# tmkhang1999/TextMAE-Image-Compression

Measured on AMD Instinct MI355X. Metric: images/sec encode+decode+rate, ViT-B 256×256 batch64, 1/2/4/8 MI355X, higher is better.
Workload: dtype bf16; 1 GPU; MCM forward eval: ids+ViT-B/16 enc (K=144 of 256 patches) + LIC hyperprior + EB/GC rates + ViT dec 512/8/16 + unpatchify; img_size=256, num_keep_patches=144, per_gpu_batch=64, global_batch=64, parallelism=replicas x1, hip_graph=True

## Files before the change

include/tmae.h:

```cpp
#ifndef TMAE_H
#define TMAE_H

#include <stdint.h>

#ifdef __cplusplus
extern "C" {
#endif

#define TMAE_ABI_VERSION 1

enum { TMAE_OK = 0, TMAE_EINVAL = 1, TMAE_EHIP = 2 };
enum { TMAE_F32 = 0, TMAE_BF16 = 1 };
enum { TMAE_ACT_NONE = 0, TMAE_ACT_GELU = 1, TMAE_ACT_RELU = 2  };

const char* tmae_last_error_string(void);
int tmae_abi_version(void);

int tmae_ids_shuffle(const float* scores, int64_t* ids_shuffle, int64_t* ids_restore, int n, int L, int K,
                     int sum_lanes, void* stream);


int tmae_layernorm_fwd(const float* x, const float* gamma, const float* beta, void* y, int rows, int D,
                       int row_group, int group_stride, int row_offset, float eps, int out_dtype, void* stream);

// ... 41 lines not shown
  int cout, act, pixel_shuffle;
  void* y; int y_f32, ldy; long long y_s1, y_s2;
  float* y32; int ld32; long long y32_s1, y32_s2;
  const float* addend; int ld_add; long long a_s1, a_s2;
  const float* lrp_src; int ld_src; long long src_s1, src_s2;
  void* y2; int ldy2; long long y2_s1, y2_s2;
  int nb1, nb2;
  void* pre; int ldp; long long pre_s1, pre_s2;
} tmae_conv_args;
int tmae_conv3x3(const tmae_conv_args* args, int dtype, void* stream);

#define TMAE_LIC_STACK_MAXL 5
typedef struct tmae_lic_stack_args {
  int n, G, nb1, nb2, nlayers;
  const void* x1; int c1, ld1; long long x1_s[2];
  const void* x2; int c2, ld2; long long x2_s[2];
  const void* w[TMAE_LIC_STACK_MAXL]; long long w_s[TMAE_LIC_STACK_MAXL][2];
  const float* bias[TMAE_LIC_STACK_MAXL]; long long b_s[TMAE_LIC_STACK_MAXL][2];
  int cout[TMAE_LIC_STACK_MAXL];
  const float* addend; int ld_add; long long a_s[2];
  void* y; int y_f32, ldy; long long y_s[2];
  const float* lrp_src; int ld_src; long long src_s[2];
  void* y2; int ldy2; long long y2_s[2];
  int flags;
  int cn; const void* cw[TMAE_LIC_STACK_MAXL]; const float* cb[TMAE_LIC_STACK_MAXL]; int ccout[TMAE_LIC_STACK_MAXL];
  const void* cx1; int cc1, cld1;
  const float* yv; int ldyv;
  const float* cadd; int cld_add;
  float* csrc; int cld_src;
  void* cy; int cldy;
  void* cy2; int cldy2;
  long long cs_x1, cs_yv, cs_src, cs_add, cs_y, cs_y2, cs_w[TMAE_LIC_STACK_MAXL], cs_b[TMAE_LIC_STACK_MAXL];
  void* sv_pre[TMAE_LIC_STACK_MAXL]; void* sv_act[TMAE_LIC_STACK_MAXL]; long long sv_s[TMAE_LIC_STACK_MAXL][2];
  float* sv_t; long long sv_t_s[2];
  void* csv_pre[TMAE_LIC_STACK_MAXL]; void* csv_act[TMAE_LIC_STACK_MAXL]; long long cs_sv[TMAE_LIC_STACK_MAXL];
  float* csv_t; long long cs_t;
  float* racc[3]; int rld[3]; int rlim[3]; long long rs[3];
  const int* cq;
} tmae_lic_stack_args;
#define TMAE_LIC_STACK_CHAIN 1
#define TMAE_LIC_STACK_BWD 2
int tmae_lic_stack(const tmae_lic_stack_args* args, void* stream);

#define TMAE_LIC_LATENT_MAXP 4
typedef struct tmae_lic_latent_args {
  int n, G, cin, nb;
  const void* x[TMAE_LIC_LATENT_MAXP]; int ldx;
  const void* w; int nfr; long long blk;
  int f_off[TMAE_LIC_LATENT_MAXP]; int f_lo, f_hi;
  float* y; int ldy;
  long long y_s[TMAE_LIC_LATENT_MAXP];
  const float* bias[TMAE_LIC_LATENT_MAXP];
  int act, y_bf16;
} tmae_lic_latent_args;
int tmae_lic_latent(const tmae_lic_latent_args* args, void* stream);

int tmae_gc_slices_fwd(const float* y, int ldy, int yoff, const float* mu, const float* sigma, long long ms_stride,
                       int ld_ms, const float* noise, float* lik, int Mtot, void* yhat, int yhat_dtype, int ld_yhat,
                       float* yhat32, int ld32, int n, int HW, int nslices, int sw, void* stream);

int tmae_gc_slices_fwd_q(const float* y, int ldy, int yoff, const float* mu, const float* sigma, long long ms_stride,
                         int ld_ms, const float* noise, float* lik, int Mtot, void* yhat, int yhat_dtype, int ld_yhat,
                         float* yhat32, int ld32, int n, int HW, int nslices, int sw, float scale_bound, const int* q,
                         void* stream);

typedef struct tmae_eb_params {
  const float* matrix[5];
  const float* bias[5];
  const float* factor[4];
  const float* quantiles;
} tmae_eb_params;

int tmae_eb_likelihood_fwd(const float* z, const tmae_eb_params* params, const float* noise, float* lik,
                           void* zhat, int zhat_dtype, float* table, int n, int C, int HW, void* stream);

int tmae_eb_aux_loss(const tmae_eb_params* params, const float* target, float* out, float* table, int C,
                     void* stream);

int tmae_gc_likelihood_fwd(const float* x, const float* scales, const float* means, const float* noise,
                           float* x_tilde, float* lik, int total, float scale_bound, void* stream);

int tmae_bpp_sum(const float* y_lik, long long ny, const float* z_lik, long long nz, double* work, float* out,
                 double num_pixels, void* stream);

int tmae_nhwc_to_nchw(const float* x, int ldx, float* y, int n, int C, int HW, void* stream);

int tmae_crop_normalize_u8(const unsigned char* src, int nsrc, int H, int W, const int* crops, int B, int S,
                           const float* mean, const float* std, float* out, void* stream);

int tmae_mae_masking(const float* noise, int64_t* ids_shuffle, int64_t* ids_restore, float* mask, int n, int L,
                     int len_keep, void* stream);

int tmae_mae_loss(const float* pred, const float* imgs, const int64_t* ids_restore, int n, int C, int H, int W, int P,
                  int len_keep, int norm_pix_loss, double* work, float* out, void* stream);

int tmae_mae_loss_bwd(const float* pred, const float* imgs, const int64_t* ids_restore, int n, int C, int H, int W,
                      int P, int len_keep, int norm_pix_loss, const float* dloss, const float* dpred_in, void* out,
                      int out_dtype, void* stream);


int tmae_gc_slices_code(const float* y, int ldy, int yoff, const float* mu, const float* sigma, long long ms_stride,
                        int ld_ms, float* lik, int Mtot, void* yhat, int yhat_dtype, int ld_yhat, float* yhat32,
                        int ld32, int n, int HW, int nslices, int sw, int* symbols, int* indexes,
                        const float* scale_table, int nscale, void* stream);

int tmae_gc_indexes(const float* sigma, long long ms_stride, int ld_ms, int n, int HW, int nslices, int sw,
// ... 252 lines not shown
```

textmae-image-compression_amd/_lib.py:

```python
from __future__ import annotations

import ctypes
import os

PKG_DIR = os.path.dirname(os.path.abspath(__file__))
LIB_PATH = os.environ.get("TMAE_LIB") or os.path.join(PKG_DIR, "lib", "libtmae.so")

TMAE_F32, TMAE_BF16 = 0, 1
ACT_NONE, ACT_GELU, ACT_RELU = 0, 1, 2

P, I, F = ctypes.c_void_p, ctypes.c_int, ctypes.c_float


LL = ctypes.c_longlong


class ConvArgs(ctypes.Structure):
    _fields_ = [
        ("x1", P), ("c1", I), ("ld1", I), ("x1_s1", LL), ("x1_s2", LL),
        ("x2", P), ("c2", I), ("ld2", I), ("x2_s1", LL), ("x2_s2", LL),
        ("n", I), ("H", I), ("W", I), ("stride", I),
        ("w", P), ("w_s1", LL), ("w_s2", LL),
        ("bias", P), ("b_s1", LL), ("b_s2", LL),
        ("cout", I), ("act", I), ("pixel_shuffle", I),
# ... 24 lines not shown
class ConvDgradArgs(ctypes.Structure):
    _fields_ = [
        ("dy", P), ("ldy", I),
        ("n", I), ("H", I), ("W", I), ("stride", I), ("cout", I), ("cin", I),
        ("wd", P),
        ("out", P), ("out_f32", I), ("ldo", I), ("pre", P), ("ldp", I),
        ("acc", P * 3), ("ld_acc", I * 3), ("lim", I * 3),
        ("nb", I), ("s_dy", LL), ("s_wd", LL), ("s_out", LL), ("s_pre", LL),
    ]


LSTK_MAXL = 5


class LicStackArgs(ctypes.Structure):
    _fields_ = [
        ("n", I), ("G", I), ("nb1", I), ("nb2", I), ("nlayers", I),
        ("x1", P), ("c1", I), ("ld1", I), ("x1_s", LL * 2),
        ("x2", P), ("c2", I), ("ld2", I), ("x2_s", LL * 2),
        ("w", P * LSTK_MAXL), ("w_s", (LL * 2) * LSTK_MAXL),
        ("bias", P * LSTK_MAXL), ("b_s", (LL * 2) * LSTK_MAXL),
        ("cout", I * LSTK_MAXL),
        ("addend", P), ("ld_add", I), ("a_s", LL * 2),
        ("y", P), ("y_f32", I), ("ldy", I), ("y_s", LL * 2),
        ("lrp_src", P), ("ld_src", I), ("src_s", LL * 2),
        ("y2", P), ("ldy2", I), ("y2_s", LL * 2),
        ("flags", I),
        ("cn", I), ("cw", P * LSTK_MAXL), ("cb", P * LSTK_MAXL), ("ccout", I * LSTK_MAXL),
        ("cx1", P), ("cc1", I), ("cld1", I),
        ("yv", P), ("ldyv", I),
        ("cadd", P), ("cld_add", I),
        ("csrc", P), ("cld_src", I),
        ("cy", P), ("cldy", I),
        ("cy2", P), ("cldy2", I),
        ("cs_x1", LL), ("cs_yv", LL), ("cs_src", LL), ("cs_add", LL), ("cs_y", LL), ("cs_y2", LL),
        ("cs_w", LL * LSTK_MAXL), ("cs_b", LL * LSTK_MAXL),
        ("sv_pre", P * LSTK_MAXL), ("sv_act", P * LSTK_MAXL), ("sv_s", (LL * 2) * LSTK_MAXL),
        ("sv_t", P), ("sv_t_s", LL * 2),
        ("csv_pre", P * LSTK_MAXL), ("csv_act", P * LSTK_MAXL), ("cs_sv", LL * LSTK_MAXL),
        ("csv_t", P), ("cs_t", LL),
        ("racc", P * 3), ("rld", I * 3), ("rlim", I * 3), ("rs", LL * 3),
        ("cq", P),
    ]


class LicLatentArgs(ctypes.Structure):
    _fields_ = [
        ("n", I), ("G", I), ("cin", I), ("nb", I),
        ("x", P * 4), ("ldx", I),
        ("w", P), ("nfr", I), ("blk", LL),
        ("f_off", I * 4), ("f_lo", I), ("f_hi", I),
        ("y", P), ("ldy", I),
        ("y_s", LL * 4), ("bias", P * 4), ("act", I), ("y_bf16", I),
    ]


class EBParams(ctypes.Structure):
    _fields_ = [("matrix", ctypes.c_void_p * 5), ("bias", ctypes.c_void_p * 5), ("factor", ctypes.c_void_p * 4),
                ("quantiles", ctypes.c_void_p)]


SIGNATURES = {
    "tmae_abi_version": [],
    "tmae_ids_shuffle": [P, P, P, I, I, I, I, P],
    "tmae_layernorm_fwd": [P, P, P, P, I, I, I, I, I, F, I, P],
    "tmae_linear_fwd": [P, I, I, I, I, I, P, P, P, I, I, P, I, I, I, I, I, I, P],
    "tmae_linear_residual_fwd": [P, I, P, P, P, I, I, I, I, I, P],
    "tmae_patch_embed_fwd": [P, P, P, P, P, P, I, I, I, I, I, I, I, I, I, P],
    "tmae_patch_embed_gathered": [P, P, P, P, P, P, I, I, I, I, I, I, P],
    "tmae_cls_rows": [P, P, P, I, I, I, P],
    "tmae_mha_fwd": [P, P, I, I, I, I, F, I, P],
    "tmae_qkv_attn_fwd": [P, P, P, P, I, I, I, I, F, I, P],
    "tmae_decoder_embed_fwd": [P, I, P, P, P, P, P, I, I, I, I, I, I, P],
    "tmae_mask_rows": [P, P, P, P, I, I, I, I, P],
    "tmae_decoder_pred_fwd": [P, P, P, P, I, I, I, I, I, I, I, I, P],
    "tmae_decoder_pred_cp_fwd": [P, P, P, P, I, I, I, I, I, I, I, I, P],
    "tmae_conv3x3": [ctypes.POINTER(ConvArgs), I, P],
    "tmae_lic_stack": [ctypes.POINTER(LicStackArgs), P],
    "tmae_lic_latent": [ctypes.POINTER(LicLatentArgs), P],
    "tmae_gc_slices_fwd": [P, I, I, P, P, LL, I, P, P, I, P, I, I, P, I, I, I, I, I, P],
    "tmae_gc_slices_fwd_q": [P, I, I, P, P, LL, I, P, P, I, P, I, I, P, I, I, I, I, I, F, P, P],
    "tmae_eb_likelihood_fwd": [P, ctypes.POINTER(EBParams), P, P, P, I, P, I, I, I, P],
    "tmae_eb_aux_loss": [ctypes.POINTER(EBParams), P, P, P, I, P],
    "tmae_gc_likelihood_fwd": [P, P, P, P, P, P, I, F, P],
    "tmae_nhwc_to_nchw": [P, I, P, I, I, I, P],
    "tmae_crop_normalize_u8": [P, I, I, I, P, I, I, ctypes.POINTER(F), ctypes.POINTER(F), P, P],
    "tmae_bpp_sum": [P, LL, P, LL, P, P, ctypes.c_double, P],
    "tmae_gemm_plan": [I, I, I, I, I, ctypes.c_char_p, I],
    "tmae_mha_plan": [I, I, I, I, ctypes.c_char_p, I],
    "tmae_mae_masking": [P, P, P, P, I, I, I, P],
    "tmae_mae_loss": [P, P, P, I, I, I, I, I, I, I, P, P, P],
    "tmae_mae_loss_bwd": [P, P, P, I, I, I, I, I, I, I, P, P, P, I, P],
    "tmae_gc_slices_code": [P, I, I, P, P, LL, I, P, I, P, I, I, P, I, I, I, I, I, P, P, P, I, P],
    "tmae_gc_indexes": [P, LL, I, I, I, I, I, P, I, F, P, P],
    "tmae_gc_dequantize": [P, P, LL, I, I, I, I, I, I, P, I, I, P, I, P],
    "tmae_gc_slices_code_q": [P, I, I, P, P, LL, I, P, I, P, I, I, P, I, I, I, I, I, P, P, P, I, F, P, P],
    "tmae_gc_indexes_q": [P, LL, I, I, I, I, I, P, I, F, P, P, P],
    "tmae_gc_dequantize_q": [P, P, LL, I, I, I, I, I, I, P, I, I, P, I, P, P],
    "tmae_gc_slices_code_qm": [P, I, I, P, P, LL, I, P, I, P, I, I, P, I, I, I, I, I, P, P, P, I, F, P, P],
    "tmae_gc_indexes_qm": [P, LL, I, I, I, I, I, P, I, F, P, P, P],
    "tmae_gc_dequantize_qm": [P, P, LL, I, I, I, I, I, I, P, I, I, P, I, P, P],
    "tmae_gc_slices_fwd_qm": [P, I, I, P, P, LL, I, P, P, I, P, I, I, P, I, I, I, I, I, F, P, P],
    "tmae_gc_pmf": [P, P, I, I, P, P, P],
    "tmae_eb_pmf": [ctypes.POINTER(EBParams), P, P, I, I, P, P, P],
    "tmae_eb_symbols": [P, ctypes.POINTER(EBParams), P, I, I, I, P, P],
    "tmae_eb_dequantize": [P, ctypes.POINTER(EBParams), P, I, I, I, P, I, P],
# ... 122 lines not shown
```

textmae-image-compression_amd/csrc/lic_stack.hip:

```cpp
#include "lic_stack_kernel.h"

int lic_stack_launch_q(const tmae_lic_stack_args& a, int nwg, hipStream_t stream);

extern "C" int tmae_lic_stack(const tmae_lic_stack_args* args, void* stream) {
  using namespace lstk;
  TMAE_REQUIRE(args != nullptr, "tmae_lic_stack: args is NULL");
  const tmae_lic_stack_args& a = *args;
  TMAE_REQUIRE(a.G >= 1 && a.G * a.G <= MAXPIX, "tmae_lic_stack: grid %dx%d exceeds %d pixels", a.G, a.G, MAXPIX);
  TMAE_REQUIRE(a.nlayers >= 1 && a.nlayers <= TMAE_LIC_STACK_MAXL, "tmae_lic_stack: %d layers", a.nlayers);
  TMAE_REQUIRE(a.nb1 >= 1 && a.nb2 >= 1 && a.n >= 1, "tmae_lic_stack: batch %d x %d, n %d", a.nb1, a.nb2, a.n);
  const bool bwd = (a.flags & TMAE_LIC_STACK_BWD) != 0;
  TMAE_REQUIRE(!a.cq || (!bwd && (a.flags & TMAE_LIC_STACK_CHAIN)),
               "tmae_lic_stack: cq (the chain's quantiser step) needs TMAE_LIC_STACK_CHAIN and no TMAE_LIC_STACK_BWD");
  TMAE_REQUIRE(a.x1 != nullptr && (a.y != nullptr || bwd), "tmae_lic_stack: x1 / y required");
  if (bwd) {
    TMAE_REQUIRE(!(a.flags & TMAE_LIC_STACK_CHAIN) && !a.addend && !a.lrp_src && !a.x2 && !a.sv_t,
                 "tmae_lic_stack: the backward chain takes no chain / addend / lrp / second source");
    const bool rt = a.racc[0] != nullptr;
    for (int l = 0; l < a.nlayers; ++l)
      TMAE_REQUIRE(a.w[l] && ((rt && l + 1 == a.nlayers) || (a.sv_pre[l] && a.sv_act[l])),
                   "tmae_lic_stack: backward layer %d needs w / sv_pre / sv_act", l);
    if (rt) {
      const int cl = a.cout[a.nlayers - 1];
      TMAE_REQUIRE(a.nb2 <= 1, "tmae_lic_stack: routed accumulators need nb2 == 1 (got %d)", a.nb2);
      TMAE_REQUIRE(a.rlim[0] >= 0 && a.rlim[0] <= a.rlim[1] && a.rlim[1] <= a.rlim[2] && a.rlim[2] == cl &&
                   a.rlim[0] % 4 == 0 && a.rlim[1] % 4 == 0, "tmae_lic_stack: routes %d / %d / %d of %d channels",
                   a.rlim[0], a.rlim[1], a.rlim[2], cl);
      for (int r = 0; r < 3; ++r)
        TMAE_REQUIRE((r == 0 ? a.rlim[0] : a.rlim[r] - a.rlim[r - 1]) == 0 || (a.racc[r] && a.rld[r] % 4 == 0),
                     "tmae_lic_stack: route %d accumulator", r);
    }
  }
  TMAE_REQUIRE(a.c1 >= 0 && a.c2 >= 0 && (a.c2 == 0 || a.x2 != nullptr), "tmae_lic_stack: channels %d + %d", a.c1, a.c2);
  TMAE_REQUIRE(a.c1 % 8 == 0 && a.c2 % 8 == 0 && a.ld1 % 8 == 0 && (a.c2 == 0 || a.ld2 % 8 == 0),
               "tmae_lic_stack: input channels / strides must be multiples of 8");
  TMAE_REQUIRE(pad32(a.c1 + a.c2) <= MAXC, "tmae_lic_stack: %d input channels exceed %d", a.c1 + a.c2, MAXC);
  for (int l = 0; l < a.nlayers; ++l) {
    TMAE_REQUIRE((a.w[l] != nullptr || (l == 0 && a.c1 + a.c2 == 0)) && (a.bias[l] != nullptr || bwd),
                 "tmae_lic_stack: layer %d weights", l);
    TMAE_REQUIRE(a.cout[l] >= 4 && a.cout[l] % 8 == 0, "tmae_lic_stack: layer %d cout %d (multiple of 8)", l, a.cout[l]);
    TMAE_REQUIRE((l + 1 == a.nlayers && (!bwd || a.racc[0])) || pad32(a.cout[l]) <= MAXC,
                 "tmae_lic_stack: layer %d cout %d exceeds %d", l, a.cout[l], MAXC);
  }
  TMAE_REQUIRE(!a.lrp_src || !a.y_f32, "tmae_lic_stack: lrp output is bf16");
  if (a.flags & TMAE_LIC_STACK_CHAIN) {
    TMAE_REQUIRE(a.nb1 == 2 && a.y_f32 && !a.lrp_src && a.cn >= 1 && a.cn <= TMAE_LIC_STACK_MAXL,
                 "tmae_lic_stack: chain needs the 2 x nb2 mean / scale problems with f32 outputs");
    TMAE_REQUIRE(a.ccout[a.cn - 1] == a.cout[a.nlayers - 1] && a.cx1 && a.yv && a.csrc && a.cy,
                 "tmae_lic_stack: chain operands");
    TMAE_REQUIRE(a.cc1 % 8 == 0 && a.cld1 % 8 == 0 && a.ldyv % 4 == 0 && a.cld_src % 4 == 0 && a.ldy % 4 == 0 &&
                 pad32(a.cc1 + a.ccout[a.cn - 1]) <= MAXC, "tmae_lic_stack: chain channels %d + %d", a.cc1,
                 a.ccout[a.cn - 1]);
    for (int l = 0; l < a.cn; ++l)
      TMAE_REQUIRE(a.cw[l] && a.cb[l] && a.ccout[l] % 8 == 0 && (l + 1 == a.cn || pad32(a.ccout[l]) <= MAXC),
                   "tmae_lic_stack: chain layer %d", l);
  }
  if (a.addend) TMAE_REQUIRE(a.ld_add % 4 == 0, "tmae_lic_stack: addend stride %d", a.ld_add);
  for (int l = 0; l < a.nlayers; ++l)
    TMAE_REQUIRE(!a.sv_pre[l] == !a.sv_act[l], "tmae_lic_stack: layer %d keeps pre-activation and output together", l);
  for (int l = 0; l < a.cn && (a.flags & TMAE_LIC_STACK_CHAIN); ++l)
    TMAE_REQUIRE(!a.csv_pre[l] == !a.csv_act[l], "tmae_lic_stack: chain layer %d keeps pre and output together", l);
  TMAE_REQUIRE(!a.sv_t || a.lrp_src, "tmae_lic_stack: sv_t is the lrp stack's pre-tanh value");
  const int nwg = a.n * a.nb1 * a.nb2;
  if (bwd) hipLaunchKernelGGL((lic_stack_kernel<true, false>), dim3(nwg), dim3(NW * 64), 0, (hipStream_t)stream, a);
  else if (a.cq) return lic_stack_launch_q(a, nwg, (hipStream_t)stream);
  else hipLaunchKernelGGL((lic_stack_kernel<false, false>), dim3(nwg), dim3(NW * 64), 0, (hipStream_t)stream, a);
  TMAE_LAUNCH_CHECK("tmae_lic_stack");
}

namespace llat {
constexpr int NW = 8, FPW = 2 * NW;
constexpr int MAXCIN = 384;
constexpr unsigned PMAX = lstk::pitch(MAXCIN);
constexpr unsigned ZOFF = lstk::MAXPIX * PMAX;
constexpr unsigned TMASK = ZOFF + 16 * PMAX;
constexpr int LDS_BYTES = TMASK + 320;
}
__device__ __forceinline__ constexpr unsigned llat_zoff() { return llat::ZOFF; }
__device__ __forceinline__ constexpr unsigned llat_tmask() { return llat::TMASK; }

struct LlatOut {
  void* y;
  int ldy, bf, act;
  const float* bias;
};

template <int NKC>
__device__ __forceinline__ void llat_item(const bf16* w, int nfr, long long blk, int f0, int fcol, bool two,
                                          const unsigned char* lb, unsigned pin, int G, int npix, int img,
                                          const LlatOut& o, int lane) {
  constexpr int MF = 9, NS = 9 * NKC;
  constexpr int D = NKC % 4 == 0 ? 4 : NKC % 3 == 0 ? 3 : NKC % 2 == 0 ? 2 : (NKC <= 7 ? NKC : 1);
  asm volatile("" : "+v"(lane));
  const int fr = lane & 15, fq = lane >> 4;
  f32x4 acc[2][MF];
#pragma unroll
  for (int i = 0; i < 2; ++i)
#pragma unroll
    for (int j = 0; j < MF; ++j) acc[i][j] = f32x4{0.f, 0.f, 0.f, 0.f};
  const unsigned sstride = (unsigned)nfr * 512u;
  const bf16* wl[2];
  bf16x8 ar[D][2];
#pragma unroll
  for (int i = 0; i < 2; ++i) {
    const int f = two || i == 0 ? f0 + i : f0;
    const int b = f / nfr, fi = f - b * nfr;
    wl[i] = w + b * blk + ((size_t)fi * 64 + lane) * 8;
#pragma unroll
    for (int d = 0; d < D; ++d) {
      ar[d][i] = *reinterpret_cast<const bf16x8*>(wl[i]);
      wl[i] += sstride;
    }
  }
  unsigned tmask[MF];
#pragma unroll
  for (int j = 0; j < MF; ++j) tmask[j] = *reinterpret_cast<const unsigned short*>(lb + llat_tmask() + 2 * (16 * j + fr));
  auto row = [&](int t, int j) -> unsigned {
    const int p = 16 * j + fr, sh = (t / 3 - 1) * G + (t % 3 - 1);
    const unsigned r = (unsigned)(p + sh);
    return ((tmask[j] >> t) & 1u ? r * pin : llat_zoff() + (r & 15u) * pin) + 16u * fq;
  };
  bf16x8 bv[2][MF];
  unsigned rb[MF];
#pragma unroll
// ... 11 lines not shown
#pragma unroll
        for (int j = 0; j < MF; ++j) bv[(kc + 1) & 1][j] = *reinterpret_cast<const bf16x8*>(lb + rb[j] + 64u * (kc + 1));
      } else if (t + 1 < 9) {
#pragma unroll
        for (int j = 0; j < MF; ++j) bv[(kc + 1) & 1][j] = *reinterpret_cast<const bf16x8*>(lb + rn[j]);
      }
      bf16x8 a0[2];
      const bool more = t * NKC + kc + D < NS;
#pragma unroll
      for (int i = 0; i < 2; ++i) {
        a0[i] = ar[kc % D][i];
        if (more) {
          ar[kc % D][i] = *reinterpret_cast<const bf16x8*>(wl[i]);
          wl[i] += sstride;
        }
      }
#pragma unroll
      for (int j = 0; j < MF; ++j)
#pragma unroll
        for (int i = 0; i < 2; ++i)
          acc[i][j] = __builtin_amdgcn_mfma_f32_16x16x32_bf16(a0[i], bv[kc & 1][j], acc[i][j], 0, 0, 0);
      __builtin_amdgcn_sched_barrier(0);
    }
    if constexpr (NKC & 1) {
#pragma unroll
      for (int j = 0; j < MF; ++j) bv[0][j] = bv[1][j];
    }
#pragma unroll
    for (int j = 0; j < MF; ++j) rb[j] = rn[j];
  }
  f32x4 bias[2];
#pragma unroll
  for (int i = 0; i < 2; ++i)
    bias[i] = o.bias ? load4f(o.bias + fcol + 16 * (two ? i : 0) + 4 * fq) : f32x4{0.f, 0.f, 0.f, 0.f};
#pragma unroll
  for (int j = 0; j < MF; ++j) {
    const int p = 16 * j + fr;
    if (p >= npix) continue;
    const size_t at = ((size_t)img * npix + p) * o.ldy + fcol + 4 * fq;
#pragma unroll
    for (int i = 0; i < 2; ++i) {
      if (i == 1 && !two) break;
      f32x4 v = acc[i][j] + bias[i];
      if (o.act == TMAE_ACT_GELU) {
        const f32x2 lo = gelu2_bf16out(v.xy), hi = gelu2_bf16out(v.zw);
        v = f32x4{lo.x, lo.y, hi.x, hi.y};
      }
      if (o.bf) store4(reinterpret_cast<bf16*>(o.y) + at + 16 * i, v);
      else store4(reinterpret_cast<float*>(o.y) + at + 16 * i, v);
    }
  }
}

template <int NKC>
__global__ void __launch_bounds__(llat::NW * 64) lic_latent_kernel(tmae_lic_latent_args a) {
  using namespace llat;
  __shared__ __attribute__((aligned(16))) uint4 lds[LDS_BYTES / 16];
  unsigned char* lb = reinterpret_cast<unsigned char*>(lds);
  const int n = a.n, G = a.G, npix = G * G, cin = 32 * NKC;
  const int t = xcd_remap(blockIdx.x, gridDim.x);
  const int tile = t / n, img = t - tile * n, prob = blockIdx.y;
  const int tid = threadIdx.x, lane = tid & 63, wave = tid >> 6;
  const unsigned pin = lstk::pitch(cin);
  for (int i = tid; i < 16 * (int)pin / 16; i += NW * 64) reinterpret_cast<uint4*>(lds)[ZOFF / 16 + i] = uint4{0, 0, 0, 0};
  for (int p = tid; p < 160; p += NW * 64) {
    unsigned m = 0;
    if (p < npix) {
      const int py = p / G, px = p - py * G;
#pragma unroll
      for (int k = 0; k < 9; ++k) {
        const int yy = py + k / 3 - 1, xx = px + k % 3 - 1;
        m |= ((unsigned)yy < (unsigned)G && (unsigned)xx < (unsigned)G) ? (1u << k) : 0u;
      }
    }
    *reinterpret_cast<unsigned short*>(lb + TMASK + 2 * p) = (unsigned short)m;
  }
  {
    const bf16* x = reinterpret_cast<const bf16*>(a.x[prob]);
    constexpr int q = 4 * NKC;
    for (int i = tid; i < npix * q; i += NW * 64) {
      const int p = i / q, ch = 8 * (i - p * q);
      *reinterpret_cast<uint4*>(lb + p * pin + 2 * ch) =
          *reinterpret_cast<const uint4*>(x + ((size_t)img * npix + p) * a.ldx + ch);
    }
  }
  __syncthreads();
  const int fr0 = a.f_lo + tile * FPW + 2 * wave;
  if (fr0 >= a.f_hi) return;
  LlatOut o;
  o.ldy = a.ldy;
  o.bf = a.y_bf16;
  o.act = a.act;
  o.bias = a.bias[prob];
  o.y = a.y_bf16 ? (void*)(reinterpret_cast<bf16*>(a.y) + a.y_s[prob]) : (void*)(a.y + a.y_s[prob]);
  llat_item<NKC>(reinterpret_cast<const bf16*>(a.w), a.nfr, a.blk, a.f_off[prob] + fr0, 16 * fr0, fr0 + 1 < a.f_hi, lb,
                 pin, G, npix, img, o, lane);
}

extern "C" int tmae_lic_latent(const tmae_lic_latent_args* args, void* stream) {
  TMAE_REQUIRE(args != nullptr, "tmae_lic_latent: args is NULL");
  const tmae_lic_latent_args& a = *args;
  TMAE_REQUIRE(a.G >= 1 && a.G * a.G <= lstk::MAXPIX, "tmae_lic_latent: grid %dx%d", a.G, a.G);
  TMAE_REQUIRE(a.cin >= 32 && a.cin % 32 == 0 && a.cin <= llat::MAXCIN, "tmae_lic_latent: cin %d (multiple of 32, <= %d)",
               a.cin, llat::MAXCIN);
  TMAE_REQUIRE(a.nb >= 1 && a.nb <= TMAE_LIC_LATENT_MAXP && a.n >= 1, "tmae_lic_latent: %d problems, %d images", a.nb,
               a.n);
  TMAE_REQUIRE(a.w && a.y && a.ldx % 8 == 0 && a.ldx >= a.cin, "tmae_lic_latent: operands / strides");
  TMAE_REQUIRE(a.nfr >= 1 && a.f_lo >= 0 && a.f_hi > a.f_lo && a.f_lo % 2 == 0, "tmae_lic_latent: fragments [%d, %d) "
               "of blocks of %d (f_lo even)", a.f_lo, a.f_hi, a.nfr);
  TMAE_REQUIRE(a.blk >= 9LL * (a.cin / 32) * a.nfr * 512 || a.f_off[0] + a.f_hi <= a.nfr, "tmae_lic_latent: block stride");
  TMAE_REQUIRE(a.act == TMAE_ACT_NONE || a.act == TMAE_ACT_GELU, "tmae_lic_latent: act %d", a.act);
  TMAE_REQUIRE(a.ldy % 4 == 0 && (a.ldy >= 16 * a.f_hi), "tmae_lic_latent: ldy %d", a.ldy);
  for (int j = 0; j < a.nb; ++j)
    TMAE_REQUIRE(a.x[j] && a.f_off[j] >= 0 && a.y_s[j] % 4 == 0, "tmae_lic_latent: problem %d", j);
  const int ntile = (a.f_hi - a.f_lo + llat::FPW - 1) / llat::FPW;
  const dim3 grid(a.n * ntile, a.nb);
  hipStream_t st = (hipStream_t)stream;
  switch (a.cin / 32) {
#define LLAT_CASE(K) \
  case K: hipLaunchKernelGGL(lic_latent_kernel<K>, grid, dim3(llat::NW * 64), 0, st, a); break;
    LLAT_CASE(1) LLAT_CASE(2) LLAT_CASE(3) LLAT_CASE(4) LLAT_CASE(5) LLAT_CASE(6)
    LLAT_CASE(7) LLAT_CASE(8) LLAT_CASE(9) LLAT_CASE(10) LLAT_CASE(11) LLAT_CASE(12)
#undef LLAT_CASE
    default: break;
  }
  TMAE_LAUNCH_CHECK("tmae_lic_latent");
}
```

textmae-image-compression_amd/mcm.py:

```python
from __future__ import annotations

import collections.abc
import os

from functools import partial

import numpy as np
import torch
import torch.nn as nn

from . import ops
from .entropy import CompressionModel, EntropyBottleneck, GaussianConditional
from .layers import Block, BlockScratch, BlockWeights, PatchEmbed, conv3x3, run_block, subpel_conv3x3
from .pos_embed import get_2d_sincos_pos_embed


class MCM(CompressionModel):

    def __init__(self, img_size=224, patch_size=16, in_chans=3, encoder_embed_dim=768, encoder_depth=12,
                 encoder_num_heads=12, decoder_embed_dim=512, decoder_depth=8, decoder_num_heads=16, mlp_ratio=4.0,
                 norm_layer=partial(nn.LayerNorm, eps=1e-6), norm_pix_loss=False, latent_depth=384,
                 hyperprior_depth=192, num_slices=12, num_keep_patches=144):
        super().__init__()
        self.frozen_stages = -1
# ... 644 lines not shown
                s1 += 1
            part = [sections[j] for j in jobs[s0:s1]]
            try:
                x_hat = self._decode_sections([a[0] for a in part], [a[1] for a in part], [a[2] for a in part],
                                              lanes[0], lanes[1], who, [index[k].q for k, _ in jobs[s0:s1]],
                                              [(index[k].nlev, index[k].offsets, a[3])
                                               for (k, _), a in zip(jobs[s0:s1], part)])
            except ValueError as e:

                def name(m, s0=s0):
                    k, t = jobs[s0 + int(m.group(1))]
                    return f"tile {t} of source {where[k]}" if many else f"tile {t}"

                raise ValueError(re.sub(r"\bimage (\d+)", name, str(e), count=1)) from None
            if tiles is None:
                tiles = torch.empty((len(jobs),) + tuple(x_hat.shape[1:]), dtype=torch.float32, device=x_hat.device)
            tiles[s0:s1].copy_(x_hat)
            s0 = s1
        images = [(g.H, g.W, slots[k]) for k, g in enumerate(grids)]
        return ops.tile_blend_crops(tiles, images, windows, size, index[0].overlap, out=out)


class _LazyStreams(collections.abc.Mapping):

    def __init__(self, **tensors):
        self._t, self._h = tensors, {}

    def __getitem__(self, key):
        if key not in self._h:
            self._h[key] = self._t[key].cpu().numpy()
        return self._h[key]

    def __iter__(self):
        return iter(self._t)

    def __len__(self):
        return len(self._t)


def _interleave(layers):
    out = []
    for j, l in enumerate(layers):
        out.append(l)
        if j < len(layers) - 1:
            out.append(nn.GELU())
    return out


class _Executor:

    USE_LIC_STACK = True
    USE_LIC_CHAIN = True
    USE_LIC_LATENT = True

    def __init__(self, m: MCM, batch, dtype, device):
        self.m, self.batch, self.dtype, self.device = m, batch, dtype, device
        self._sig = None
        B = batch
        E, Dd, M, N, S = m.encoder_embed_dim, m.decoder_embed_dim, m.latent_depth, m.hyperprior_depth, m.num_slices
        K = m.num_keep_patches
        P = m.encoder_embed.patch_size[0]
        self.img = m.encoder_embed.img_size[0]
        self.P, self.L = P, m.encoder_embed.num_patches
        self.g = g = int(round(K ** 0.5))
        if g * g != K:
            raise ValueError(f"num_keep_patches={K} must be a perfect square (MCM.py:729-732 views it as sqrt x sqrt)")
        self.hz = ((g + 1) // 2 + 1) // 2
        if self.hz * 4 != g:
            raise ValueError(f"sqrt(num_keep_patches)={g} must be a multiple of 4 so h_s returns to the y grid")
        self.sw = M // S
        self.maxsup = S // 2
        gc = m.gaussian_conditional
        self.scale_bound = float(gc.scale_bound) if gc.scale_bound is not None else 0.11
        self.nb = S - self.maxsup
        f32, dt = torch.float32, dtype
        dev = device

        def z(*shape, dtype=f32):
            return torch.empty(shape, dtype=dtype, device=dev)

        Te, Td = K + 1, self.L + 1
        Mp = B * g * g
        self.Mp = Mp
        hid_e = m.encoder_blocks[0].mlp.fc1.out_features if m.encoder_depth else 4 * E
        hid_d = m.decoder_blocks[0].mlp.fc1.out_features if m.decoder_depth else 4 * Dd
        self.tok = z(B * Te, E)
        self.enc_s = BlockScratch(B * Te, E, hid_e, dt, dev)
        self.enc_out = z(B * K, E, dtype=dt)
        ga = [l.out_channels for l in m.g_a if isinstance(l, nn.Conv2d)]
        self.ga_buf = [z(B * K, c, dtype=dt) for c in ga[:-1]]
        self.Y32 = z(Mp, M)
        self.YT = self.Y32 if dt == f32 else z(Mp, M, dtype=dt)
        ha = [l.out_channels for l in m.h_a if isinstance(l, nn.Conv2d)]
        res = [g, g, (g + 1) // 2, (g + 1) // 2, self.hz]
        self.ha_buf = [z(B * r * r, c, dtype=dt) for c, r in zip(ha[:-1], res[:-1])]
        self.Z = z(B * self.hz * self.hz, N)
        self.ZLIK = z(B, N, self.hz, self.hz)
        self.ZHAT = z(B * self.hz * self.hz, N, dtype=dt)
        self.eb_table = z(N, 59)
        self.zero_loss = torch.zeros((), device=device)
        hs_out = [m.h_s_mean[0].out_channels, m.h_s_mean[2][0].out_channels // 4, m.h_s_mean[4].out_channels,
                  m.h_s_mean[6][0].out_channels // 4]
        hs_res = [self.hz, 2 * self.hz, 2 * self.hz, g]
        self.hs_buf = [z(2, B * r * r, c, dtype=dt) for c, r in zip(hs_out, hs_res)]
        self.LSM = z(2, Mp, M, dtype=dt)
        self.LS, self.LM = self.LSM[0], self.LSM[1]
        self.mid = [l.out_channels for l in m.cc_transform_mean[0] if isinstance(l, nn.Conv2d)]
        c0 = self.mid[0]
        self.PW = 3 * S * c0
        self.Pbuf = z(Mp, self.PW)
        self.overlap = torch.device(dev).type == "cuda"
        self.side_stream = torch.cuda.Stream(device=dev) if self.overlap else None
        self.SUPY = z(Mp, M, dtype=dt)
        self.YPRE = z(Mp, M)
        self.YH = z(Mp, M, dtype=dt)
        nb = self.nb
        self.CM = [z(2, nb, Mp, c, dtype=dt) for c in self.mid[:-1]]
        self.MUSIG = z(2, nb, Mp, self.sw)
        self.MS_SER = z(2, S, Mp, self.sw)
        self.CL = [z(nb, Mp, c, dtype=dt) for c in self.mid[:-1]]
        self.YLIK = z(B, M, g, g)
        gs = [l.out_channels for l in m.g_s if isinstance(l, nn.ConvTranspose2d)]
        self.gs_buf = [z(B * K, c, dtype=dt) for c in gs]
        self.dec = z(B * Td, Dd)
        self.dec_s = BlockScratch(B * Td, Dd, hid_d, dt, dev)
        self.dn = z(B * self.L, Dd, dtype=dt)

    def refresh_weights(self):
        sig = tuple((p.data_ptr(), p._version) for p in self.m.parameters())
        if sig == self._sig:
            return
        self._sig = sig
        m, dt = self.m, self.dtype
        M, S, sw, ms = m.latent_depth, m.num_slices, self.sw, self.maxsup

        def cast(t):
            t = t.detach()
            return (t if dt == torch.float32 else t.to(dt)).contiguous()

        def cw(w, lo=None, hi=None):
            w = w.detach()
            if lo is not None:
                w = w[:, lo:hi]
            return w.permute(0, 2, 3, 1).reshape(w.shape[0], -1)

        self.w_pe = cast(m.encoder_embed.proj.weight.view(m.encoder_embed.proj.weight.shape[0], -1))
        self.enc_w = [BlockWeights.from_block(b, dt) for b in m.encoder_blocks]
        self.dec_w = [BlockWeights.from_block(b, dt) for b in m.decoder_blocks]
        self.ga_w = [(cast(l.weight.view(l.weight.shape[0], -1)), l.bias.detach())
                     for l in m.g_a if isinstance(l, nn.Conv2d)]
        self.gs_w = [(cast(l.weight.view(l.weight.shape[0], -1).t()), l.bias.detach())
                     for l in m.g_s if isinstance(l, nn.ConvTranspose2d)]
        self.ha_w = [(cast(cw(l.weight)), l.bias.detach(), l.stride[0]) for l in m.h_a if isinstance(l, nn.Conv2d)]

        def hs_convs(seq):
            out = []
            for l in seq:
                if isinstance(l, nn.Conv2d):
                    out.append((l, False))
                elif isinstance(l, nn.Sequential):
                    out.append((l[0], True))
            return out

        self.hs2_w = [(cast(torch.stack([cw(s.weight), cw(mn.weight)])),
                       torch.stack([s.bias, mn.bias]).detach().contiguous(), ps)
# ... 478 lines not shown
                ops.gc_slices_code_q(self.Y32, M, i0 * sw, mu, sigma, ms_stride, sw, None, M, self.SUPY, dt, M,
                                     self.YPRE, M, B, HW, nbs, sw, sym[i0 * per:], idx[i0 * per:], table, bound, qd)
        return step

    def _gc_decompress(self, decoder):
        gc = self.m.gaussian_conditional
        M, sw, B, HW, dt = self.m.latent_depth, self.sw, self.batch, self.g * self.g, self.dtype
        cdf, sizes, offsets = gc.host_tables()
        bound = float(gc.scale_bound) if gc.scale_bound is not None else 0.11
        per = B * sw * HW
        idx_dev = torch.empty(self.m.num_slices * per, dtype=torch.int32, device=self.device)

        def step(i0, nbs, mu, sigma, ms_stride):
            n = nbs * per
            ops.gc_indexes(sigma, ms_stride, sw, B, HW, nbs, sw, gc.scale_table, bound, idx_dev)
            idx = idx_dev[:n].cpu().numpy()
            vals = decoder.decode_stream_array(idx, cdf, sizes, offsets)
            sym = torch.from_numpy(vals).to(self.device)
            ops.gc_dequantize(sym, mu, ms_stride, sw, B, HW, nbs, sw, i0 * sw, self.SUPY, dt, M, self.YPRE, M)
        return step

    def _h_s(self):
        B, dt = self.batch, self.dtype
        x, xs, cin, H = self.ZHAT, 0, self.m.hyperprior_depth, self.hz
        for j, (w, b, pshuf) in enumerate(self.hs2_w):
            last = j == len(self.hs2_w) - 1
            cout = w.shape[1]
            out = self.LSM if last else self.hs_buf[j]
            ops.conv3x3(x, cin, cin, B, H, H, w, b, out, out.shape[2], cout, dt,
                        act=ops.ACT_NONE if last else ops.ACT_GELU, pixel_shuffle=pshuf, nb=(1, 2),
                        strides={"x1": (0, xs), "w": (0, w[0].numel()), "b": (0, cout), "y": (0, out[0].numel())})
            if pshuf:
                H *= 2
                cin = cout // 4
            else:
                cin = cout
            x, xs = out, out[0].numel()

    def _slices(self, gc_step, chain_ok=False, cq=None):
        m, dt, B, g = self.m, self.dtype, self.batch, self.g
        M, S, sw, ms, nb, Mp = m.latent_depth, m.num_slices, self.sw, self.maxsup, self.nb, self.Mp
        mid = self.mid
        c0 = mid[0]
        Pw = self.PW
        Pb = self.Pbuf
        eP = Pb.element_size()
        pbase = Pb.data_ptr()
        off_mean, off_lrp, off_scale = 0, S * c0, 2 * S * c0
        esz = self.SUPY.element_size()
        supy, ypre, yh = self.SUPY.data_ptr(), self.YPRE.data_ptr(), self.YH.data_ptr()
        e4 = 4
        wrow = self.w_pre_ml[0].numel()

        def pre(i0, i1):
            if self.w_lat is not None:
                nfs = c0 // 16
                ops.lic_latent(B, g, [self.LM, self.LM, self.LS], M, M, self.w_lat, nfs, self.w_lat[0].numel(),
                               [0, S * nfs, 2 * S * nfs], i0 * nfs, i1 * nfs, pbase, Pw)
                return
            n = (i1 - i0) * c0
            ops.conv3x3(self.LM, M, M, B, g, g, self.w_pre_ml[i0 * c0:], None, pbase + (off_mean + i0 * c0) * eP, Pw,
                        n, dt, y_f32=True, nb=(1, 2), strides={"w": (0, S * c0 * wrow), "y": (0, S * c0)})
            ops.conv3x3(self.LS, M, M, B, g, g, self.w_pre_s[i0 * c0:], None, pbase + (off_scale + i0 * c0) * eP,
                        Pw, n, dt, y_f32=True)

        ready = {}
        groups = [(i, i + 1) for i in range(1, ms)] + ([(ms, S)] if nb > 0 else [])
        if self.overlap and groups:
            main = torch.cuda.current_stream()
            pre(0, 1)
            fork = torch.cuda.Event()
            fork.record(main)
            side = self.side_stream
            side.wait_event(fork)
            with torch.cuda.stream(side):
                for i0, i1 in groups:
                    pre(i0, i1)
                    ev = torch.cuda.Event()
                    ev.record(side)
                    ready[i0] = ev
        else:
            pre(0, S)

        def wait_pre(i0):
            if i0 in ready:
                torch.cuda.current_stream().wait_event(ready.pop(i0))

        cm = [t.data_ptr() for t in self.CM]
        cl = [t.data_ptr() for t in self.CL]
        musig = self.MUSIG.data_ptr()
        cm_s1 = [nb * Mp * c for c in mid[:-1]]
        ms_s1 = nb * Mp * sw

        def ms_stack(first, layers, x1, c1, i0, nbs):
            w, b = first
            ops.conv3x3(x1, c1, M, B, g, g, w, b, cm[0], c0, c0, dt, act=ops.ACT_GELU,
                        addend=pbase + (off_mean + i0 * c0) * eP, ld_add=Pw, nb=(2, nbs),
                        strides={"w": (w[0].numel(), w[0][0].numel() if nbs > 1 else 0),
                                 "b": (b[0].numel(), c0 if nbs > 1 else 0),
                                 "a": (off_scale - off_mean, c0), "y": (cm_s1[0], Mp * c0)})
            for j, (w, b) in enumerate(layers):
                cin, cout = mid[j], mid[j + 1]
                last = j == len(layers) - 1
                y = musig if last else cm[j + 1]
                ys1 = ms_s1 if last else cm_s1[j + 1]
                ops.conv3x3(cm[j], cin, cin, B, g, g, w, b, y, cout, cout, dt,
                            act=ops.ACT_NONE if last else ops.ACT_GELU, y_f32=last, nb=(2, nbs),
                            strides={"x1": (cm_s1[j], Mp * cin), "w": (w[0].numel(), w[0][0].numel() if nbs > 1 else 0),
                                     "b": (b[0].numel(), cout if nbs > 1 else 0), "y": (ys1, Mp * cout)})

        def ms_fused(i0, nbs):
            ws = self.lstk["b_ms"] if nbs > 1 else self.lstk["ms"][i0]
            first, layers = (self.b_ms_first, self.b_ms_layers) if nbs > 1 else (self.ms_first[i0], self.ms_layers[i0])
            bs_ = [first[1]] + [b for _, b in layers]
            st = {"a": (off_scale - off_mean, c0), "y": (ms_s1, Mp * sw)}
            for l, (w, b) in enumerate(zip(ws, bs_)):
                st[f"w{l}"] = (w[0].numel(), w[0][0].numel() if nbs > 1 else 0)
                st[f"b{l}"] = (b[0].numel(), b.shape[-1] if nbs > 1 else 0)
            ops.lic_stack(B, g, supy, sw * (ms if nbs > 1 else i0), M, ws, bs_, mid, musig, sw, True,
                          addend=pbase + (off_mean + i0 * c0) * eP, ld_add=Pw, nb=(2, nbs), strides=st)

        def lrp_fused(i0, nbs):
            ws = self.lstk["b_lrp"] if nbs > 1 else self.lstk["lrp"][i0]
            first, layers = (self.b_lrp_first, self.b_lrp_layers) if nbs > 1 else (self.lrp_first[i0], self.lrp_layers[i0])
            bs_ = [first[1]] + [b for _, b in layers]
            st = {"a": (0, c0), "y": (0, sw), "src": (0, sw), "x2": (0, sw)}
            for l, (w, b) in enumerate(zip(ws, bs_)):
                st[f"w{l}"] = (0, w[0].numel() if nbs > 1 else 0)
                st[f"b{l}"] = (0, b.shape[-1] if nbs > 1 else 0)
            if nbs > 1:
# ... 83 lines not shown
```

textmae-image-compression_amd/ops.py:

```python
from __future__ import annotations

import contextlib
import ctypes
import os

import torch

from . import _lib
from ._lib import ACT_GELU, ACT_NONE, TMAE_BF16, TMAE_F32, ConvArgs, EBParams, LicStackArgs

__all__ = [
    "ids_shuffle", "layernorm", "linear", "linear_residual", "patch_embed", "cls_rows", "mha", "decoder_embed",
    "mask_rows", "decoder_pred", "conv3x3", "lic_stack", "pack_lic_stack_weight", "lic_stack_fits", "gc_slices", "eb_likelihood", "eb_aux_loss",
    "gc_likelihood", "nhwc_to_nchw", "bpp", "gemm_plan", "force_gemm_tile", "GEMM_TILES", "mha_plan", "mha_force_stream", "dtype_code", "gc_slices_code", "gc_indexes",
    "gc_dequantize", "gc_slices_fwd_q", "gc_slices_code_q", "gc_indexes_q", "gc_dequantize_q",
    "gc_slices_fwd_qm", "gc_slices_code_qm", "gc_indexes_qm", "gc_dequantize_qm",
    "qlevels_select", "qlevels_pack", "qlevels_unpack", "qmap_build",
    "gc_pmf", "eb_pmf", "eb_symbols", "eb_dequantize", "invert_permutation", "mae_masking",
    "rans_stream_cap_words", "rans_encode_streams", "rans_pack_streams", "rans_decode_streams",
    "rans_encode_lanes", "rans_decode_lanes", "ids_pack", "ids_unpack",
    "resize_tables", "resize_u8", "rgb_to_gray_u8", "tile_cut_u8", "tile_blend", "tile_blend_crops",
    "mae_loss", "TMAE_F32", "TMAE_BF16", "ACT_NONE", "ACT_GELU",
]

# ... 237 lines not shown
    if ci:
        t[:, :co, :ci] = w.float().permute(2, 3, 0, 1).reshape(9, co, ci)
    nkc, nfr = cip // 32, cop // 16
    t = t.view(9, nfr, 16, nkc, 4, 8).permute(0, 3, 1, 4, 2, 5).contiguous()
    return t.view(-1).to(dtype)


def pack_lic_stack_weight_t(w: torch.Tensor, dtype=torch.bfloat16) -> torch.Tensor:
    return pack_lic_stack_weight(w.detach().transpose(0, 1).flip(2, 3), dtype)


def lic_stack_bwd(n, G, dtop, ldt, c_top, weights, couts, pres, outs, nb=(1, 1), strides=None, routes=None):
    a = LicStackArgs()
    if routes is not None:
        if nb[1] != 1:
            raise ValueError("lic_stack_bwd routes: nb2 must be 1")
        if len(routes) > 1 and len(routes) != nb[0]:
            raise ValueError("lic_stack_bwd routes: one route list per problem")
        lim = 0
        for r in range(3):
            if r < len(routes[0]):
                acc, ld, nc = routes[0][r]
                a.racc[r], a.rld[r] = _p(acc), ld
                if len(routes) > 1 and nc:
                    steps = [_p(routes[k + 1][r][0]) - _p(routes[k][r][0]) for k in range(len(routes) - 1)]
                    if len(set(steps)) != 1 or steps[0] % 4:
                        raise ValueError("lic_stack_bwd routes: accumulators not at a constant stride")
                    a.rs[r] = steps[0] // 4
                lim += nc
            a.rlim[r] = lim
    a.n, a.G, a.nlayers = n, G, len(couts)
    a.nb1, a.nb2 = nb
    a.x1, a.c1, a.ld1 = _p(dtop), c_top, ldt
    a.flags = 2
    for l, (w, c) in enumerate(zip(weights, couts)):
        a.w[l], a.cout[l] = _p(w), c
        if l < len(pres):
            a.sv_pre[l], a.sv_act[l] = _p(pres[l]), _p(outs[l])
    for name, (s1, s2) in (strides or {}).items():
        if name[0] == "w":
            a.w_s[int(name[1:])][:] = (s1, s2)
        elif name[0] == "s":
            a.sv_s[int(name[1:])][:] = (s1, s2)
        else:
            getattr(a, f"{name}_s")[:] = (s1, s2)
    _lib.call("tmae_lic_stack", ctypes.byref(a), _stream())


def lic_latent_fits(G, cin):
    return G * G <= LSTK_MAXPIX and cin % 32 == 0 and 32 <= cin <= 384


def lic_latent(n, G, xs, ldx, cin, w, nfr, blk, f_off, f_lo, f_hi, y, ldy, y_s=None, biases=None, act=ACT_NONE,
               y_bf16=False):
    a = _lib.LicLatentArgs()
    a.n, a.G, a.cin, a.nb = n, G, cin, len(xs)
    for j, (x, fo) in enumerate(zip(xs, f_off)):
        a.x[j] = _p(x)
        a.f_off[j] = fo
        a.y_s[j] = (16 * fo) if y_s is None else y_s[j]
        a.bias[j] = _p(biases[j]) if biases is not None else None
    a.ldx, a.w, a.nfr, a.blk = ldx, _p(w), nfr, blk
    a.f_lo, a.f_hi = f_lo, f_hi
    a.y, a.ldy = _p(y), ldy
    a.act, a.y_bf16 = act, int(y_bf16)
    _lib.call("tmae_lic_latent", ctypes.byref(a), _stream())


def lic_stack(n, G, x1, c1, ld1, weights, biases, couts, y, ldy, y_f32, x2=None, c2=0, ld2=0, addend=None, ld_add=0,
              lrp_src=None, ld_src=0, y2=None, ldy2=0, nb=(1, 1), strides=None, chain=None, save=None):
    a = LicStackArgs()
    a.n, a.G, a.nlayers = n, G, len(couts)
    a.nb1, a.nb2 = nb
    a.x1, a.c1, a.ld1 = _p(x1), c1, ld1
    a.x2, a.c2, a.ld2 = _p(x2), c2, ld2
    for l, (w, b, c) in enumerate(zip(weights, biases, couts)):
        a.w[l], a.bias[l], a.cout[l] = _p(w), _p(b), c
    a.addend, a.ld_add = _p(addend), ld_add
    a.y, a.y_f32, a.ldy = _p(y), int(y_f32), ldy
    a.lrp_src, a.ld_src = _p(lrp_src), ld_src
    a.y2, a.ldy2 = _p(y2), ldy2
    if chain is not None:
        a.flags = 1
        a.cn = len(chain["couts"])
        for l, (w, b, c) in enumerate(zip(chain["w"], chain["b"], chain["couts"])):
            a.cw[l], a.cb[l], a.ccout[l] = _p(w), _p(b), c
        a.cx1, a.cc1, a.cld1 = _p(chain["x1"]), chain["c1"], chain["ld1"]
        a.yv, a.ldyv = _p(chain["y"]), chain["ldy"]
        a.cadd, a.cld_add = _p(chain["add"]), chain["ld_add"]
        a.csrc, a.cld_src = _p(chain["ypre"]), chain["ld_ypre"]
        a.cy, a.cldy = _p(chain["out"]), chain["ld_out"]
        a.cy2, a.cldy2 = _p(chain.get("out2")), chain.get("ld_out2", 0)
        a.cq = _q_ptr(chain.get("q"), n)
        cs = chain.get("strides", {})
        a.cs_x1, a.cs_yv, a.cs_src = cs.get("x1", 0), cs.get("y", 0), cs.get("ypre", 0)
        a.cs_add, a.cs_y, a.cs_y2 = cs.get("add", 0), cs.get("out", 0), cs.get("out2", 0)
        for l in range(a.cn):
            a.cs_w[l], a.cs_b[l] = cs.get(f"w{l}", 0), cs.get(f"b{l}", 0)
    for name, (s1, s2) in (strides or {}).items():
        if name[0] in "wb" and name[1:].isdigit():
            getattr(a, f"{name[0]}_s")[int(name[1:])][:] = (s1, s2)
        else:
            getattr(a, f"{name}_s")[:] = (s1, s2)
    if save is not None:
        for l, (pre, act, st) in enumerate(save.get("layers", [])):
            a.sv_pre[l], a.sv_act[l] = _p(pre), _p(act)
            a.sv_s[l][:] = st
        if save.get("t") is not None:
            a.sv_t = _p(save["t"])
            a.sv_t_s[:] = save.get("t_s", (0, 0))
        for l, (pre, act, st) in enumerate(save.get("chain", [])):
            a.csv_pre[l], a.csv_act[l] = _p(pre), _p(act)
            a.cs_sv[l] = st
        if save.get("chain_t") is not None:
            a.csv_t, a.cs_t = _p(save["chain_t"]), save.get("chain_t_s", 0)
    _lib.call("tmae_lic_stack", ctypes.byref(a), _stream())


# ... 673 lines not shown
```

Baseline: 10130 images/s.

## Make lic_latent a persistent CU-capped kernel sharing input staging across problems

The latent-prior kernel goes from one workgroup per (tile, image, problem) to a persistent grid sized to the CU count, optionally capped when running on the side stream. Each workgroup walks a contiguous range of frame-pair work units, and problems that read the same input tensor are grouped so the image is staged into LDS once and reused. A host-side search picks a grid size that minimises the worst-case number of rounds, memoised per shape. The goal is to cut redundant LDS staging and to leave CUs free for the overlapping main-stream work. The cost is less parallelism per launch and extra index arithmetic inside the kernel.

```diff
diff --git a/include/tmae.h b/include/tmae.h
--- a/include/tmae.h
+++ b/include/tmae.h
@@ -117,6 +117,7 @@
   long long y_s[TMAE_LIC_LATENT_MAXP];
   const float* bias[TMAE_LIC_LATENT_MAXP];
   int act, y_bf16;
+  int max_wg;
 } tmae_lic_latent_args;
 int tmae_lic_latent(const tmae_lic_latent_args* args, void* stream);
 
diff --git a/textmae-image-compression_amd/_lib.py b/textmae-image-compression_amd/_lib.py
--- a/textmae-image-compression_amd/_lib.py
+++ b/textmae-image-compression_amd/_lib.py
@@ -100,6 +100,7 @@
         ("f_off", I * 4), ("f_lo", I), ("f_hi", I),
         ("y", P), ("ldy", I),
         ("y_s", LL * 4), ("bias", P * 4), ("act", I), ("y_bf16", I),
+        ("max_wg", I),
     ]
 
 
diff --git a/textmae-image-compression_amd/csrc/lic_stack.hip b/textmae-image-compression_amd/csrc/lic_stack.hip
--- a/textmae-image-compression_amd/csrc/lic_stack.hip
+++ b/textmae-image-compression_amd/csrc/lic_stack.hip
@@ -69,7 +69,7 @@
 }
 
 namespace llat {
-constexpr int NW = 8, FPW = 2 * NW;
+constexpr int NW = 8;
 constexpr int MAXCIN = 384;
 constexpr unsigned PMAX = lstk::pitch(MAXCIN);
 constexpr unsigned ZOFF = lstk::MAXPIX * PMAX;
@@ -187,16 +187,28 @@
   }
 }
 
+__device__ __forceinline__ int llat_lane() {
+  int l;
+  asm volatile("v_mbcnt_lo_u32_b32 %0, -1, 0\n\tv_mbcnt_hi_u32_b32 %0, -1, %0" : "=v"(l));
+  return l;
+}
+
+struct LlatPlan {
+  int nmap, npair, units;
+  int mprob[TMAE_LIC_LATENT_MAXP];
+  int mbeg[TMAE_LIC_LATENT_MAXP + 1];
+};
+
 template <int NKC>
-__global__ void __launch_bounds__(llat::NW * 64) lic_latent_kernel(tmae_lic_latent_args a) {
+__global__ void __launch_bounds__(llat::NW * 64) lic_latent_kernel(tmae_lic_latent_args a, LlatPlan pl) {
   using namespace llat;
   __shared__ __attribute__((aligned(16))) uint4 lds[LDS_BYTES / 16];
   unsigned char* lb = reinterpret_cast<unsigned char*>(lds);
   const int n = a.n, G = a.G, npix = G * G, cin = 32 * NKC;
-  const int t = xcd_remap(blockIdx.x, gridDim.x);
-  const int tile = t / n, img = t - tile * n, prob = blockIdx.y;
-  const int tid = threadIdx.x, lane = tid & 63, wave = tid >> 6;
+  const int tid = threadIdx.x, wave = __builtin_amdgcn_readfirstlane(tid >> 6);
   const unsigned pin = lstk::pitch(cin);
+  int u = (int)((long long)blockIdx.x * pl.units / gridDim.x);
+  const int u1 = (int)((long long)(blockIdx.x + 1) * pl.units / gridDim.x);
   for (int i = tid; i < 16 * (int)pin / 16; i += NW * 64) reinterpret_cast<uint4*>(lds)[ZOFF / 16 + i] = uint4{0, 0, 0, 0};
   for (int p = tid; p < 160; p += NW * 64) {
     unsigned m = 0;
@@ -210,26 +222,88 @@
     }
     *reinterpret_cast<unsigned short*>(lb + TMASK + 2 * p) = (unsigned short)m;
   }
-  {
-    const bf16* x = reinterpret_cast<const bf16*>(a.x[prob]);
-    constexpr int q = 4 * NKC;
-    for (int i = tid; i < npix * q; i += NW * 64) {
-      const int p = i / q, ch = 8 * (i - p * q);
-      *reinterpret_cast<uint4*>(lb + p * pin + 2 * ch) =
-          *reinterpret_cast<const uint4*>(x + ((size_t)img * npix + p) * a.ldx + ch);
-    }
-  }
-  __syncthreads();
-  const int fr0 = a.f_lo + tile * FPW + 2 * wave;
-  if (fr0 >= a.f_hi) return;
-  LlatOut o;
-  o.ldy = a.ldy;
-  o.bf = a.y_bf16;
-  o.act = a.act;
-  o.bias = a.bias[prob];
-  o.y = a.y_bf16 ? (void*)(reinterpret_cast<bf16*>(a.y) + a.y_s[prob]) : (void*)(a.y + a.y_s[prob]);
-  llat_item<NKC>(reinterpret_cast<const bf16*>(a.w), a.nfr, a.blk, a.f_off[prob] + fr0, 16 * fr0, fr0 + 1 < a.f_hi, lb,
-                 pin, G, npix, img, o, lane);
+  int m = 0, mbase = 0;
+  bool resident = false;
+  while (u < u1) {
+    int vp = (pl.mbeg[m + 1] - pl.mbeg[m]) * pl.npair;
+    while (u >= mbase + n * vp) {
+      mbase += n * vp;
+      ++m;
+      vp = (pl.mbeg[m + 1] - pl.mbeg[m]) * pl.npair;
+    }
+    const int img = (u - mbase) / vp, q0 = u - mbase - img * vp, q1 = min(vp, q0 + (u1 - u));
+    if (resident) __syncthreads();
+    resident = true;
+    {
+      const bf16* x = reinterpret_cast<const bf16*>(a.x[pl.mprob[pl.mbeg[m]]]);
+      constexpr int q = 4 * NKC;
+      const int t0 = 64 * wave + llat_lane();
+      for (int i = t0; i < npix * q; i += NW * 64) {
+        const int p = i / q, ch = 8 * (i - p * q);
+        *reinterpret_cast<uint4*>(lb + p * pin + 2 * ch) =
+            *reinterpret_cast<const uint4*>(x + ((size_t)img * npix + p) * a.ldx + ch);
+      }
+    }
+    __syncthreads();
+    for (int q = q0 + wave; q < q1; q += NW) {
+      const int pi = q / pl.npair, prob = pl.mprob[pl.mbeg[m] + pi];
+      const int fr0 = a.f_lo + 2 * (q - pi * pl.npair);
+      LlatOut o;
+      o.ldy = a.ldy;
+      o.bf = a.y_bf16;
+      o.act = a.act;
+      o.bias = a.bias[prob];
+      o.y = a.y_bf16 ? (void*)(reinterpret_cast<bf16*>(a.y) + a.y_s[prob]) : (void*)(a.y + a.y_s[prob]);
+      llat_item<NKC>(reinterpret_cast<const bf16*>(a.w), a.nfr, a.blk, a.f_off[prob] + fr0, 16 * fr0,
+                     fr0 + 1 < a.f_hi, lb, pin, G, npix, img, o, llat_lane());
+    }
+    u += q1 - q0;
+  }
+}
+
+namespace llat {
+static int max_rounds(const int* vp, int n, long long U, int W) {
+  int worst = 0, m = 0;
+  long long base = 0;
+  for (int w = 0; w < W; ++w) {
+    long long u = w * U / W;
+    const long long u1 = (w + 1) * U / W;
+    int r = 0;
+    while (u < u1) {
+      while (u >= base + (long long)n * vp[m]) base += (long long)n * vp[m++];
+      const long long q0 = (u - base) % vp[m], len = std::min<long long>(vp[m] - q0, u1 - u);
+      r += (int)((len + NW - 1) / NW);
+      u += len;
+    }
+    worst = std::max(worst, r);
+  }
+  return worst;
+}
+
+static int pick_grid(const int* vp, int nmap, int n, long long U, int cap) {
+  cap = (int)std::min<long long>(cap, U);
+  if (cap <= 1 || (long long)nmap * n > 4096) return std::max(cap, 1);
+  struct Memo { int vp[TMAE_LIC_LATENT_MAXP], nmap, n, cap, W; };
+  constexpr int NMEMO = 16;
+  thread_local Memo memo[NMEMO];
+  thread_local int nmemo = 0, next = 0;
+  for (int i = 0; i < nmemo; ++i) {
+    const Memo& e = memo[i];
+    if (e.nmap == nmap && e.n == n && e.cap == cap && std::equal(vp, vp + nmap, e.vp)) return e.W;
+  }
+  int best = cap, rbest = max_rounds(vp, n, U, cap);
+  const int floor_r = (int)((U + (long long)cap * NW - 1) / ((long long)cap * NW));
+  for (int W = cap - 1; W >= std::max(1, cap / 2) && rbest > floor_r; --W) {
+    const int r = max_rounds(vp, n, U, W);
+    if (r < rbest) best = W, rbest = r;
+  }
+  Memo& e = memo[next];
+  next = (next + 1) % NMEMO;
+  nmemo = std::min(nmemo + 1, NMEMO);
+  std::copy(vp, vp + nmap, e.vp);
+  e.nmap = nmap, e.n = n, e.cap = cap, e.W = best;
+  return best;
+}
 }
 
 extern "C" int tmae_lic_latent(const tmae_lic_latent_args* args, void* stream) {
@@ -248,12 +322,34 @@
   TMAE_REQUIRE(a.ldy % 4 == 0 && (a.ldy >= 16 * a.f_hi), "tmae_lic_latent: ldy %d", a.ldy);
   for (int j = 0; j < a.nb; ++j)
     TMAE_REQUIRE(a.x[j] && a.f_off[j] >= 0 && a.y_s[j] % 4 == 0, "tmae_lic_latent: problem %d", j);
-  const int ntile = (a.f_hi - a.f_lo + llat::FPW - 1) / llat::FPW;
-  const dim3 grid(a.n * ntile, a.nb);
+  TMAE_REQUIRE(a.max_wg >= 0, "tmae_lic_latent: max_wg %d", a.max_wg);
+  LlatPlan pl = {};
+  pl.npair = (a.f_hi - a.f_lo + 1) / 2;
+  const long long units = (long long)a.n * a.nb * pl.npair;
+  TMAE_REQUIRE(units < (1LL << 30), "tmae_lic_latent: %lld pair units", units);
+  pl.units = (int)units;
+  int vp[TMAE_LIC_LATENT_MAXP];
+  for (int j = 0, k = 0; j < a.nb; ++j) {
+    bool head = true;
+    for (int i = 0; i < j; ++i) head = head && a.x[i] != a.x[j];
+    if (!head) continue;
+    const int k0 = k;
+    for (int i = j; i < a.nb; ++i)
+      if (a.x[i] == a.x[j]) pl.mprob[k++] = i;
+    pl.mbeg[pl.nmap] = k0;
+    vp[pl.nmap] = (k - k0) * pl.npair;
+    pl.mbeg[++pl.nmap] = k;
+  }
+  int dev = 0, cus = 0;
+  TMAE_REQUIRE(hipGetDevice(&dev) == hipSuccess &&
+               hipDeviceGetAttribute(&cus, hipDeviceAttributeMultiprocessorCount, dev) == hipSuccess && cus >= 1,
+               "tmae_lic_latent: the device's CU count");
+  const int cap = a.max_wg > 0 ? std::min(a.max_wg, cus) : cus;
+  const dim3 grid(llat::pick_grid(vp, pl.nmap, a.n, units, cap));
   hipStream_t st = (hipStream_t)stream;
   switch (a.cin / 32) {
 #define LLAT_CASE(K) \
-  case K: hipLaunchKernelGGL(lic_latent_kernel<K>, grid, dim3(llat::NW * 64), 0, st, a); break;
+  case K: hipLaunchKernelGGL(lic_latent_kernel<K>, grid, dim3(llat::NW * 64), 0, st, a, pl); break;
     LLAT_CASE(1) LLAT_CASE(2) LLAT_CASE(3) LLAT_CASE(4) LLAT_CASE(5) LLAT_CASE(6)
     LLAT_CASE(7) LLAT_CASE(8) LLAT_CASE(9) LLAT_CASE(10) LLAT_CASE(11) LLAT_CASE(12)
 #undef LLAT_CASE
diff --git a/textmae-image-compression_amd/mcm.py b/textmae-image-compression_amd/mcm.py
--- a/textmae-image-compression_amd/mcm.py
+++ b/textmae-image-compression_amd/mcm.py
@@ -720,6 +720,7 @@
     USE_LIC_STACK = True
     USE_LIC_CHAIN = True
     USE_LIC_LATENT = True
+    LATENT_SIDE_BUDGET = True
 
     def __init__(self, m: MCM, batch, dtype, device):
         self.m, self.batch, self.dtype, self.device = m, batch, dtype, device
@@ -779,6 +780,10 @@
         self.Pbuf = z(Mp, self.PW)
         self.overlap = torch.device(dev).type == "cuda"
         self.side_stream = torch.cuda.Stream(device=dev) if self.overlap else None
+        self.side_wg = 0
+        if self.overlap and self.LATENT_SIDE_BUDGET:
+            cus = torch.cuda.get_device_properties(dev).multi_processor_count
+            self.side_wg = max(cus - 2 * B, cus // 4)
         self.SUPY = z(Mp, M, dtype=dt)
         self.YPRE = z(Mp, M)
         self.YH = z(Mp, M, dtype=dt)
@@ -1363,11 +1368,11 @@
         e4 = 4
         wrow = self.w_pre_ml[0].numel()
 
-        def pre(i0, i1):
+        def pre(i0, i1, max_wg=0):
             if self.w_lat is not None:
                 nfs = c0 // 16
                 ops.lic_latent(B, g, [self.LM, self.LM, self.LS], M, M, self.w_lat, nfs, self.w_lat[0].numel(),
-                               [0, S * nfs, 2 * S * nfs], i0 * nfs, i1 * nfs, pbase, Pw)
+                               [0, S * nfs, 2 * S * nfs], i0 * nfs, i1 * nfs, pbase, Pw, max_wg=max_wg)
                 return
             n = (i1 - i0) * c0
             ops.conv3x3(self.LM, M, M, B, g, g, self.w_pre_ml[i0 * c0:], None, pbase + (off_mean + i0 * c0) * eP, Pw,
@@ -1386,7 +1391,7 @@
             side.wait_event(fork)
             with torch.cuda.stream(side):
                 for i0, i1 in groups:
-                    pre(i0, i1)
+                    pre(i0, i1, self.side_wg)
                     ev = torch.cuda.Event()
                     ev.record(side)
                     ready[i0] = ev
diff --git a/textmae-image-compression_amd/ops.py b/textmae-image-compression_amd/ops.py
--- a/textmae-image-compression_amd/ops.py
+++ b/textmae-image-compression_amd/ops.py
@@ -313,7 +313,7 @@
 
 
 def lic_latent(n, G, xs, ldx, cin, w, nfr, blk, f_off, f_lo, f_hi, y, ldy, y_s=None, biases=None, act=ACT_NONE,
-               y_bf16=False):
+               y_bf16=False, max_wg=0):
     a = _lib.LicLatentArgs()
     a.n, a.G, a.cin, a.nb = n, G, cin, len(xs)
     for j, (x, fo) in enumerate(zip(xs, f_off)):
@@ -324,7 +324,7 @@
     a.ldx, a.w, a.nfr, a.blk = ldx, _p(w), nfr, blk
     a.f_lo, a.f_hi = f_lo, f_hi
     a.y, a.ldy = _p(y), ldy
-    a.act, a.y_bf16 = act, int(y_bf16)
+    a.act, a.y_bf16, a.max_wg = act, int(y_bf16), max_wg
     _lib.call("tmae_lic_latent", ctypes.byref(a), _stream())
 
 
```

Measured after the change: 10200 images/s, median of 6. Within noise of the previous version (+0.7%).
